# terminusdb-labs/parallel-hnsw

Hardware: AMD Instinct MI355X
Metric: queries/sec at recall@10≥0.95 on 1M×768 f32 (higher is better)
Workload: dtype f32

## Files before the change

### parallel_hnsw_amd/csrc/api.hip

```cpp
#include <hip/hip_runtime.h>

#include <algorithm>
#include <atomic>
#include <cmath>
#include <cstdarg>
#include <cstdio>
#include <cstring>
#include <new>
#include <stdexcept>
#include <vector>

#include "exact_slices.h"
#include "phnsw_internal.h"

static thread_local std::string g_err;

void ph_set_error(const char *fmt, ...) {
  char buf[1024];
  va_list ap;
  va_start(ap, fmt);
  vsnprintf(buf, sizeof(buf), fmt, ap);
  va_end(ap);
  g_err = buf;
}
// ... 674 lines not shown
      int rc = ph_layer_anchor_pos(mix->store, mix->layers[a.n_layers - 1]);
      if (rc) return rc;
      a.probe_pos = mix->layers[a.n_layers - 1].pos;
    }
  }
#endif
#ifdef PH_VISITED_PROBE
  {
    static unsigned long long *vprobe_dev = nullptr;
    if (!vprobe_dev) {
      PH_HIP(hipMalloc(&vprobe_dev, 130 * sizeof(unsigned long long)));
      PH_HIP(hipMemset(vprobe_dev, 0, 130 * sizeof(unsigned long long)));
    } else {
      unsigned long long h[130];
      PH_HIP(hipDeviceSynchronize());
      PH_HIP(hipMemcpy(h, vprobe_dev, sizeof(h), hipMemcpyDeviceToHost));
      for (int k = 0; k < 2; k++) {
        unsigned long long n = 0, sum = 0, run = 0;
        for (int b = 0; b < 64; b++) n += h[64 * k + b], sum += h[64 * k + b] * (64ull * b + 32ull);
        if (!n) continue;
        fprintf(stderr, "[visited probe] %s: %llu walks, mean ~%.0f ids, past the LDS load limit: %.4f; ids < 64*(b+1) for",
                k ? "bottom layer" : "upper gathered layers", n, (double)sum / (double)n, (double)h[128 + k] / (double)n);
        for (int b = 0; b < 64; b++) {
          run += h[64 * k + b];
          if (h[64 * k + b]) fprintf(stderr, " b%d:%.4f", b, (double)run / (double)n);
        }
        fprintf(stderr, "\n");
      }
      PH_HIP(hipMemset(vprobe_dev, 0, 130 * sizeof(unsigned long long)));
    }
    a.vprobe_out = vprobe_dev;
  }
#endif
  return 0;
}

int ph_search_device(const phnsw_index *ix, const PhSearchCall &c) {
  phnsw_index *mix = const_cast<phnsw_index *>(ix);
  const uint64_t nq = c.nq;
  const uint32_t knn_mode = c.knn_mode, out_stride = c.out_stride;
  uint32_t *const out_index = c.out_index;
  const hipStream_t stream = c.stream;
  if (ph_store_converted(ix->store) && (knn_mode || out_index || c.hint || c.out_hit)) {
    return ph_search_only_unsupported(ix->store, knn_mode ? "knn / threshold_nn" : (out_index ? "search_instrumented" : "build search"));
  }
  PhSearchArgs a;
  fill_args(ix, c, a);
  if (ix->dbg_order && ix->dbg_order_n == nq) a.order = ix->dbg_order;
  std::lock_guard<std::mutex> g(mix->ws_mutex);
  if (!mix->totals) {
    PH_HIP(hipMalloc(&mix->totals, 16));
    PH_HIP(hipMemset(mix->totals, 0, 16));
  }
  a.totals = mix->totals;
  PhWorkspace &ws = mix->ws[mix->ws_next & 1];
  mix->ws_last = mix->ws_next & 1;
  mix->ws_next++;
  int rc = ph_workspace_ensure(ix, ws, std::max(a.ef, a.cap_max), c.ovf_cap ? c.ovf_cap : default_ovf_cap(a.ef));
  if (rc) return rc;
  const uint32_t T = (knn_mode || out_index) ? 0u : ph_tiny_layer_count(ix, a.n_layers, a.ef);
  uint32_t first_big = a.n_layers;
  for (uint32_t l = std::max(1u, T); l < a.n_layers; l++)
    if (ph_layer_own_launch(ix->layers[l].n_nodes, ph_row_bytes(ix->store))) {
      first_big = l;
      break;
    }
// ... 337 lines not shown
    return PHNSW_E_INVALID;
  }
  PhFilter f;
  int rc = ph_filter_check(ix, filter_dev, filter_stride_words, 0u, call, &f);
  if (rc) return rc;
  if (!f.words) f.words = ix->default_filter;
  PH_HIP(hipSetDevice(ix->store->device));
  return ph_filter_count(ix, f, nbitmaps, out_count_dev, (hipStream_t)stream);
} catch (...) { return ph_caught(); }

extern "C" int phnsw_debug_last_tiny_table(const phnsw_index *ix, float *out_host, uint64_t cap_floats, uint32_t *npos,
                                           uint32_t *tn, uint32_t *stride, int *g) try {
  if (!ix) return PHNSW_E_INVALID;
  phnsw_index *mix = const_cast<phnsw_index *>(ix);
  std::lock_guard<std::mutex> lock(mix->ws_mutex);
  PhWorkspace &ws = mix->ws[mix->ws_last];
  if (!ws.timed || !ws.d_tiny || !ws.tiny_d) {
    ph_set_error("the last search on this index made no dense table");
    return PHNSW_E_INVALID;
  }
  const uint64_t need = (uint64_t)ws.tiny_last_npos * ws.tiny_last_stride;
  if (npos) *npos = ws.tiny_last_npos;
  if (tn) *tn = ws.tiny_last_tn;
  if (stride) *stride = ws.tiny_last_stride;
  if (g) *g = ws.tiny_table_g;
  if (out_host) {
    if (cap_floats < need) {
      ph_set_error("phnsw_debug_last_tiny_table: %llu floats needed", (unsigned long long)need);
      return PHNSW_E_INVALID;
    }
    PH_HIP(hipSetDevice(ix->store->device));
    PH_HIP(hipEventSynchronize(ws.ev1));
    PH_HIP(hipMemcpy(out_host, ws.tiny_d, need * 4u, hipMemcpyDeviceToHost));
  }
  return 0;
} catch (...) { return ph_caught(); }

extern "C" int phnsw_debug_layer_pos(phnsw_index *ix, uint32_t lft, uint32_t *out_host) try {
  if (lft >= ix->layers.size() || !ix->layers[lft].pos) return PHNSW_E_INVALID;
  PH_HIP(hipMemcpy(out_host, ix->layers[lft].pos, (size_t)ix->layers[lft].n_nodes * 4, hipMemcpyDeviceToHost));
  return 0;
} catch (...) { return ph_caught(); }

extern "C" int phnsw_debug_set_order(phnsw_index *ix, const uint32_t *order_dev, uint64_t n) try {
  ix->dbg_order = order_dev;
  ix->dbg_order_n = n;
  return 0;
} catch (...) { return ph_caught(); }

extern "C" int phnsw_index_counters(const phnsw_index *ix, uint64_t *n_dist, uint64_t *n_hops) try {
  if (!ix) return PHNSW_E_INVALID;
  unsigned long long h[2] = {0, 0};
  if (ix->totals) {
    PH_HIP(hipSetDevice(ix->store->device));
    PH_HIP(hipDeviceSynchronize());
    PH_HIP(hipMemcpy(h, ix->totals, 16, hipMemcpyDeviceToHost));
  }
  if (n_dist) *n_dist = h[0];
  if (n_hops) *n_hops = h[1];
  return 0;
} catch (...) { return ph_caught(); }

extern "C" int phnsw_last_search_kernel_ms(const phnsw_index *ix, float *ms) try {
  if (!ix || !ms) return PHNSW_E_INVALID;
  phnsw_index *mix = const_cast<phnsw_index *>(ix);
  std::lock_guard<std::mutex> g(mix->ws_mutex);
// ... 340 lines not shown
```

### parallel_hnsw_amd/csrc/phnsw_internal.h

```cpp
#pragma once
#include <hip/hip_runtime.h>
#include <stdint.h>
#include <stdlib.h>

#include <mutex>
#include <string>
#include <vector>

#include "../../include/phnsw.h"

#define PH_EMPTY32 0xFFFFFFFFu
#define PH_FMAX 3.4028234663852886e38f
#define PH_MAX_LAYERS 24
#define PH_WAVE 64
#define PH_MAX_DISPATCH 24
#define PH_DENSE_SPLIT_MIN 2048u
#define PH_TINY_MAX_NODES 8192u
#define PH_TINY_LDS_NODES 1024u
#define PH_TINY_MAX_LAYERS 8

void ph_set_error(const char *fmt, ...);
int ph_caught() noexcept;
int ph_hip_fail(hipError_t e, const char *what, const char *file, int line);
#define PH_HIP(x)                                                       \
// ... 59 lines not shown
};

struct phnsw_store {
  int device = 0;
  int kind = PH_ROWS_F32;
  float *rows = nullptr;
  uint8_t *codes = nullptr;
  uint16_t *codes16 = nullptr;
  phnsw_store *centroid_store = nullptr;
  phnsw_index *centroid_index = nullptr;
  phnsw_search_params quantized_search = {0, 0, 0};
  float *codebook = nullptr;
  uint32_t pq_m = 0, pq_ksub = 0, pq_dsub = 0;
  uint32_t pq_table_f16 = 0;
  void *packed = nullptr;
  uint32_t packed_stride = 0;
  float *anchors = nullptr;
  uint32_t *anchor_rank = nullptr;
  uint32_t n_anchors = 0;
  bool owns_rows = true;
  uint64_t n = 0;
  uint32_t dim = 0, ld = 0;
  int metric = 0;
  int refcount = 1;
};

struct PhTinyPrepKey {
  bool valid = false;
  uint64_t nodes_epoch = 0;
  uint32_t T = 0, tn = 0;
  const void *nodes[PH_TINY_MAX_LAYERS] = {}, *nbrs[PH_TINY_MAX_LAYERS] = {}, *vec2node = nullptr;
  uint32_t n[PH_TINY_MAX_LAYERS] = {}, W[PH_TINY_MAX_LAYERS] = {};
  uint64_t links[PH_TINY_MAX_LAYERS] = {};
};
struct PhTinyPackKey {
  bool valid = false;
  uint64_t nodes_epoch = 0;
  const void *vecs = nullptr, *tnodes = nullptr;
  uint32_t ld = 0, tn = 0, nv = 0;
};

struct PhWorkspace {
  uint32_t *visited = nullptr;
  uint64_t visited_words = 0;
  uint2 *ovf = nullptr;
  uint32_t ovf_cap = 0;
  uint32_t n_slots = 0;
  uint32_t *counter = nullptr;
  hipEvent_t ev0 = nullptr, ev1 = nullptr;
  hipEvent_t evc = nullptr;
  bool timed = false;
  void *pq_tables = nullptr;
  size_t pq_tables_bytes = 0;
  uint32_t *okey = nullptr, *okey_sorted = nullptr, *oiota = nullptr, *oorder = nullptr;
  void *sort_tmp = nullptr;
  size_t sort_tmp_bytes = 0;
  uint32_t order_cap = 0;
  float *tiny_d = nullptr;
  size_t tiny_d_bytes = 0;
  uint32_t *tiny_nbr = nullptr;
  size_t tiny_nbr_bytes = 0;
  uint32_t *tiny_member = nullptr;
  size_t tiny_member_bytes = 0;
  float4 *tiny_pq = nullptr, *tiny_pn = nullptr;
  size_t tiny_pq_bytes = 0, tiny_pn_bytes = 0;
  PhTinyPrepKey tiny_prep_key;
  PhTinyPackKey tiny_pack_key;
  int tiny_table_g = 0;
  uint32_t tiny_last_npos = 0, tiny_last_tn = 0, tiny_last_stride = 0;
  uint2 *dense_ovf = nullptr;
  size_t dense_ovf_bytes = 0;
  uint32_t *ovf_s = nullptr;
  size_t ovf_s_cap = 0;
  uint32_t *park_ids = nullptr;
  float *park_d = nullptr;
  size_t park_ids_bytes = 0, park_d_bytes = 0;
  hipEvent_t evd[PH_MAX_DISPATCH + 1] = {};
  unsigned long long *dtotals = nullptr;
  uint32_t n_dispatch = 0;
  uint32_t n_chunks = 0;
  int cus = 0;
  uint32_t d_lo[PH_MAX_DISPATCH] = {}, d_hi[PH_MAX_DISPATCH] = {};
  bool d_tiny = false;
};

struct PhBuildTable {
  float *D = nullptr;
  size_t bytes = 0;
  size_t cap = 0;
  const uint32_t *qnodes = nullptr, *tnodes = nullptr;
  uint32_t qn = 0, tn = 0, T = 0, stride = 0;
  uint32_t lo_alloc = 0, hi_alloc = 0, lo = 0, hi = 0;
  uint64_t epoch = 0;
};
struct PhRowHint {
  const uint32_t *qnodes;
// ... 88 lines not shown
  void *pq_tables;
  uint32_t pq_table_bytes;
  uint32_t layer_lo, layer_hi;
  uint32_t *out_key;
  const uint32_t *key_pos;
  uint32_t dense_only, after_dense;
  const uint32_t *dense_flag;
  uint2 *dense_ovf;
  uint32_t dense_ovf_cap;
#ifdef PH_CELL_PROBE
  const uint32_t *probe_pos;
  unsigned long long *probe_out;
#endif
#ifdef PH_VISITED_PROBE
  unsigned long long *vprobe_out;
#endif
  uint32_t vis_slots, vis_limit, vis_off;
  const uint32_t *order;
  uint32_t seg;
  uint32_t *out_hit;
  uint32_t *out_index;
  uint32_t *ovf_s;
  uint32_t tiny_layers, tiny_n, tiny_stride;
  const float *tiny_d;
  const uint32_t *tiny_nbr;
  const uint32_t *tiny_member;
  uint32_t tiny_rows, tiny_row_first;
  const uint32_t *tiny_row_map;
  uint32_t tiny_off[PH_TINY_MAX_LAYERS];
  const uint32_t *label_of, *label_want;
  uint32_t collect_k, collect_flags;
  uint32_t *collect_ids;
  float *collect_d;
};

uint32_t ph_default_ovf_cap(uint32_t ef);
hipError_t ph_timed_malloc(void **p, size_t bytes);
hipError_t ph_timed_free(void *p);
#ifndef PH_RAW_ALLOC
#define hipMalloc(p, n) ph_timed_malloc((void **)(p), (n))
#define hipFree(p) ph_timed_free((void *)(p))
#endif
static inline long long env_ll(const char *name) {
  const char *e = getenv(name);
  return e ? atoll(e) : 0;
}
static inline uint32_t grid1(uint64_t items) {
  const uint64_t blocks = (items + 255u) / 256u;
  return (uint32_t)(blocks < (1u << 16) ? blocks : (1u << 16));
}
int ph_stream_beside(hipStream_t other, hipStream_t *io);
hipError_t ph_pool_alloc(void **p, size_t bytes);
void ph_pool_free(void *p);
void ph_pool_trim(void);
void ph_layer_free(PhLayerHost &l);
void ph_pending_free(phnsw_index *ix);
void ph_host_stages_free(phnsw_index *ix);
int ph_layer_upload(phnsw_index *ix, const uint32_t *nodes, const uint32_t *neighbors, uint32_t n, uint32_t W,
                    PhLayerHost *out);
struct PhSearchCall {
  const float *queries;
  uint32_t ldq;
  const uint32_t *qids, *exclude;
  uint64_t nq;
  const phnsw_search_params *sp;
  uint32_t upto;
// ... 234 lines not shown
```

### parallel_hnsw_amd/csrc/search_kernels.h

```cpp
#pragma once
#include <hip/hip_runtime.h>

#include <algorithm>
#include <cstdio>
#include <cstdlib>
#include <cstring>

#include "phnsw_internal.h"

#include "phnsw_device.h"

#ifdef PH_HOP_PROFILE
#define PH_TICK(k)                                   \
  {                                                  \
    asm volatile("s_waitcnt vmcnt(0) lgkmcnt(0)");   \
    const uint64_t t_now = wall_clock64();           \
    tprof[k] += t_now - t_last;                      \
    t_last = t_now;                                  \
  }
#else
#define PH_TICK(k)
#endif

template <bool BIG>
// ... 43 lines not shown
  constexpr int CAP = CAPC * 64;
  constexpr int FM = FILT & (PH_FM_BITMAP | PH_FM_LABEL);
  constexpr bool COLLECT = (FILT & PH_FM_COLLECT) != 0;
  constexpr int TAILF = COLLECT ? PH_FM_NONE : FM;
  uint32_t *Cid = smem;
  float *Cd = (float *)(smem + CAP);
  uint32_t *Qid = smem + 2 * CAP;
  float *Qd = (float *)(smem + 3 * CAP);
  if constexpr (BIG) {
    Qid = a.big_q + (uint64_t)blockIdx.x * 2u * a.cap_max;
    Qd = (float *)(Qid + a.cap_max);
  }
  uint32_t *S = smem + 4 * CAP;
  float *dist_lds = (float *)(smem + 5 * CAP + 64);
  if (Dist::GLOBAL_TABLE) dist_lds = (float *)((char *)a.pq_tables + (size_t)blockIdx.x * a.pq_table_bytes);
  const uint32_t T = (a.tiny_layers && a.tiny_member[a.tiny_n] == 0u) ? a.tiny_layers : 0u;
  const bool tiny_lds_row = a.tiny_n <= a.tiny_lds_nodes;
  float *Dl = (float *)(smem + 5 * CAP + 64);
  uint32_t *Vl = smem + 5 * CAP + 64 + (tiny_lds_row ? a.tiny_stride : 0u);
  const uint32_t tiny_words = (a.tiny_n + 31u) / 32u;

  const uint32_t lane = threadIdx.x;
  const uint64_t lt = lanemask_lt(lane);
  constexpr bool DENSE_ONLY = dist_is_none<Dist>::value;
  const bool table_ok = (a.dense_only || a.after_dense) ? a.dense_flag[0] == 0u : true;
  if (DENSE_ONLY && !table_ok) return;
  const uint32_t layer_lo = a.after_dense ? (table_ok ? a.after_dense : 0u) : a.layer_lo;
  uint32_t *vis = a.visited + (uint64_t)blockIdx.x * a.visited_words;
  uint2 *ovf = DENSE_ONLY ? a.dense_ovf + (uint64_t)blockIdx.x * a.dense_ovf_cap : a.ovf + (uint64_t)blockIdx.x * a.ovf_cap;
  const uint32_t ovf_cap = DENSE_ONLY ? a.dense_ovf_cap : a.ovf_cap;
  uint32_t *const Qs = S;
  uint32_t *const ovf_s = INSTR ? a.ovf_s + (uint64_t)blockIdx.x * a.ovf_cap : nullptr;
  uint32_t *const H = smem + a.vis_off;
  const uint32_t hslots = (BIG || INSTR || !vis_lds_policy<CAPC, Dist>::value) ? 0u : a.vis_slots;
  for (uint32_t i = lane; i < hslots; i += 64) H[i] = PH_EMPTY32;

  uint32_t seg_cur = 0, seg_done = 0;
  if (a.order) {
    uint32_t xcc;
    asm volatile("s_getreg_b32 %0, hwreg(HW_REG_XCC_ID)" : "=s"(xcc));
    seg_cur = (xcc & 15u) & 7u;
  }

  for (;;) {
    uint32_t q = 0, qpos = 0;
    if (!a.order) {
      if (lane == 0) q = atomicAdd(a.counter, 1u);
      q = rfl32(q);
      if (q >= a.nq) break;
      qpos = q;
    } else {
      for (;;) {
        uint32_t p = 0;
        if (lane == 0) p = atomicAdd(a.counter + seg_cur * 16u, 1u);
        p = rfl32(p);
        const uint32_t base = seg_cur * a.seg;
        const uint32_t len = base >= a.nq ? 0u : min(a.seg, a.nq - base);
        if (p < len) {
          qpos = base + p;
          q = a.order[qpos];
          break;
        }
        seg_cur = (seg_cur + 1u) & 7u;
        if (++seg_done == 8u) {
          q = PH_EMPTY32;
          break;
        }
      }
// ... 49 lines not shown
      klen = min(kk, klen + (uint32_t)__popcll(em));
      return true;
    };
    uint32_t n_dist = 0, n_hops = 0, err = ST_OK;
    uint32_t index_distance = 0xFFFFFFFFu;
    uint32_t n_tab = 0;
    uint32_t n_dist0 = 0, n_hops0 = 0;
    uint32_t clen = 0;
    uint32_t ef = a.ef;
    bool big_written = false;

    if (layer_lo) {
      clen = a.out_len[q];
#pragma unroll
      for (int c = 0; c < CAPC; c++) {
        uint32_t i = lane + 64u * c;
        if (i < clen) {
          Cid[i] = a.out_ids[(uint64_t)q * a.ef + i];
          Cd[i] = a.out_d[(uint64_t)q * a.ef + i];
        }
      }
      if (a.out_stats) {
        n_dist = a.out_stats[2 * (uint64_t)q];
        n_hops = a.out_stats[2 * (uint64_t)q + 1];
      }
      n_dist0 = n_dist;
      n_hops0 = n_hops;
    } else if (!a.knn_mode) {
      uint32_t entry = a.layers[0].nodes[0];
      float d0;
      if constexpr (DENSE_ONLY) {
        const PhLayerDev TLy = a.layers[a.tiny_layers - 1];
        const uint32_t tid = TLy.vec2node ? TLy.vec2node[entry] : entry;
        d0 = (a.tiny_d + trow * a.tiny_stride)[tid < a.tiny_n ? tid : 0u];
      } else {
        d0 = dist.batch(a.dist, 1ull, entry, lane);
      }
      d0 = __uint_as_float(rl32(__float_as_uint(d0), 0));
      n_dist = 1;
      if (lane == 0) {
        Cid[0] = entry;
        Cd[0] = d0;
      }
      clen = 1;
    }
    const float *Dg = a.tiny_d + trow * a.tiny_stride;
    if (T) {
      if (tiny_lds_row)
        for (uint32_t i = lane; i < a.tiny_n; i += 64) Dl[i] = Dg[i];
      for (uint32_t i = lane; i < tiny_words; i += 64) Vl[i] = 0u;
    }
    queue_sync<BIG>();

    for (uint32_t li = a.knn_mode ? last_layer : layer_lo; li < layer_hi && err == ST_OK; li++) {
      PhLayerDev L = a.layers[li];
      const bool tl = li < T;
      if (tl) {
        const PhLayerDev TLy = a.layers[T - 1];
        L.n_nodes = a.tiny_n;
        L.nodes = TLy.nodes;
        L.vec2node = TLy.vec2node;
        L.neighbors = a.tiny_nbr + a.tiny_off[li];
      }
      const bool identity = L.vec2node == nullptr;
      bool hv = hslots && !tl;
      uint32_t hn = 0;
      auto visit = [&](uint32_t id, bool valid) -> bool {
        if (hv && hn + (uint32_t)__popcll(__ballot(valid)) > a.vis_limit) {
          for (uint32_t i = lane; i < hslots; i += 64) {
            const uint32_t o = H[i];
            if (o != PH_EMPTY32) {
              atomicOr(&vis[o >> 5], 1u << (o & 31));
              H[i] = PH_EMPTY32;
            }
          }
          wait_vm0();
          hv = false;
        }
        if (hv) {
          const bool f = vis_insert(H, hslots, id, valid);
          hn += (uint32_t)__popcll(__ballot(f));
          return f;
        }
        if (!valid) return false;
        const uint32_t bit = 1u << (id & 31);
        return !(atomicOr(&vis[id >> 5], bit) & bit);
      };
      uint32_t qlen;
      if (a.knn_mode) {
        if (lane == 0) {
          Qid[0] = qnode;
          Qd[0] = 0.0f;
        }
        visit(qnode, lane == 0);
        qlen = 1;
// ... 111 lines not shown
            uint32_t id = __hip_atomic_load(&ovf[i].x, __ATOMIC_RELAXED, __HIP_MEMORY_SCOPE_AGENT);
            if (!(id & EXPF)) {
              uint32_t db = __hip_atomic_load(&ovf[i].y, __ATOMIC_RELAXED, __HIP_MEMORY_SCOPE_AGENT);
              uint64_t k = mkkey(__uint_as_float(db), id);
              if (k < best) {
                best = k;
                bi = i;
              }
            }
          }
#pragma unroll
          for (int s = 32; s >= 1; s >>= 1) {
            uint64_t o = ((uint64_t)__shfl_xor((uint32_t)(best >> 32), s) << 32) | __shfl_xor((uint32_t)best, s);
            uint32_t oi = __shfl_xor(bi, s);
            if (o < best) {
              best = o;
              bi = oi;
            }
          }
          if (best == KEY_NONE) break;
          cur = (uint32_t)best & IDM;
          if (lane == 0)
            __hip_atomic_store(&ovf[bi].x, cur | EXPF, __ATOMIC_RELAXED, __HIP_MEMORY_SCOPE_AGENT);
          pop = -1 - (int)bi;
        }
        uint32_t cur_s = 0;
        if constexpr (INSTR) cur_s = pop >= 0 ? Qs[pop] : ovf_s[(uint32_t)(-1 - pop)];
        cur &= IDM;
        n_hops++;
        PH_TICK(0)

        uint32_t nb = PH_EMPTY32;
        if (lane < L.W) nb = L.neighbors[(uint64_t)cur * L.W + lane];
        if constexpr (Dist::EARLY) {
          const bool valid = nb < L.n_nodes;
          uint32_t v = 0;
          if (valid) v = identity ? nb : L.nodes[nb];
          dist.prefetch(a.dist, valid, v, lane);
        }
        PH_TICK(1)
        bool fresh = false;
        if (tl) {
          if (nb < L.n_nodes) {
            uint32_t bit = 1u << (nb & 31);
            fresh = !(atomicOr(&Vl[nb >> 5], bit) & bit);
          }
        } else {
          fresh = visit(nb, nb < L.n_nodes);
        }
        const uint64_t fm = __ballot(fresh);
        const uint32_t m = __popcll(fm);
        n_dist += m;
        if (tl) n_tab += m;
#ifdef PH_CELL_PROBE
        if (probing) {
          uint32_t dd = 0xFFFFFFFFu;
          if (fresh) {
            const int d0 = (int)a.probe_pos[nb] - (int)probe_p0;
            dd = (uint32_t)(d0 < 0 ? -d0 : d0);
          }
#pragma unroll
          for (int k = 0; k < 10; k++) probe_cnt[k] += __popcll(__ballot(fresh && dd <= (k ? (1u << (k - 1)) : 0u)));
          probe_cnt[10] += m;
        }
#endif
        PH_TICK(2)
        uint32_t cvec = 0;
        bool cq = false;
        if constexpr (COLLECT) {
          if (li == last_layer && fresh) {
            cvec = identity ? nb : L.nodes[nb];
            cq = cvec != excl && passes(cvec);
          }
        }

        float myd;
        if (tl) {
          myd = 0.f;
          if (fresh) myd = tiny_lds_row ? Dl[nb] : Dg[nb];
        } else if constexpr (Dist::EARLY) {
          myd = dist.finish(a.dist, fm, lane);
        } else {
          uint32_t vid = 0;
          if (fresh) vid = identity ? nb : L.nodes[nb];
          myd = dist.batch(a.dist, fm, vid, lane);
        }

        PH_TICK(3)
        const uint64_t key = fresh ? mkkey(myd, nb) : KEY_NONE;
        uint32_t my_s = 0;
        if constexpr (INSTR) {
          uint32_t rank_all = 0;
          uint64_t remf = fm;
          while (remf) {
            const int j = __builtin_ctzll(remf);
            remf &= remf - 1;
            rank_all += (rl64(key, j) < key) ? 1u : 0u;
          }
          my_s = cur_s + rank_all + 1u;
        }
        const bool full = qlen == ef;
        const float dtail = full ? Qd[ef - 1] : PH_FMAX;
        const uint64_t tailkey = full ? mkkey(dtail, Qid[ef - 1]) : KEY_NONE;
        const bool ins = fresh && key < tailkey && myd <= PH_FMAX;
        const uint64_t im = __ballot(ins);
        uint32_t pos = 0, pos_min = 0xFFFFFFFFu, newpos = 0xFFFFFFFFu;
        bool did = im != 0;
        if (!im && m >= 2) did = __ballot(fresh && myd == dtail) != 0;
        if (im) {
          uint32_t rank = 0, greater = 0;
          bool first_pass = true;
          const int c_top = (int)((qlen - 1u) >> 6);
// ... 265 lines not shown
      for (int c = 0; c < CAPC; c++) {
        uint32_t j = lane + 64u * c;
        bool has = j < blen;
        bv[c] = has ? Qid[j] : PH_EMPTY32;
        bd[c] = has ? Qd[j] : PH_FMAX;
        bpos[c] = PH_EMPTY32;
        if (has) {
          uint32_t la = lds_lower_bound(Cid, Cd, clen, mkkey(bd[c], bv[c]));
          uint32_t dupb = la < clen ? S[la] : S[CAP];
          if (la == clen) dupb = dups;
          bpos[c] = j + (la - dupb);
        }
      }
      queue_sync<BIG>();
#pragma unroll
      for (int c = 0; c < CAPC; c++) {
        if (cpos[c] < ef) {
          Cid[cpos[c]] = ci[c];
          Cd[cpos[c]] = cd[c];
        }
        if (bpos[c] < ef) {
          Cid[bpos[c]] = bv[c];
          Cd[bpos[c]] = bd[c];
        }
      }
      clen = min(ef, clen - dups + blen);
      queue_sync<BIG>();
    }

    if (err != ST_OK) {
      if (!DENSE_ONLY)
        for (uint64_t w = lane; w < a.visited_words; w += 64) vis[w] = 0u;
      for (uint32_t i = lane; i < hslots; i += 64) H[i] = PH_EMPTY32;
      wait_vm0();
      clen = 0;
      kq = KEY_NONE;
      klen = 0;
    }
    if (TAILF && (a.filter_flags & PHNSW_FILTER_STRICT) && layer_hi == a.n_layers && !big_written) {
      uint32_t sv[CAPC];
      float sd[CAPC];
      uint32_t spos[CAPC];
      uint32_t kept = 0;
#pragma unroll
      for (int c = 0; c < CAPC; c++) {
        const uint32_t i = lane + 64u * c;
        const bool has = i < clen;
        sv[c] = has ? Cid[i] : 0u;
        sd[c] = has ? Cd[i] : PH_FMAX;
        bool keep = false;
        if (has) keep = passes(sv[c]);
        const uint64_t km = __ballot(keep);
        spos[c] = keep ? kept + __popcll(km & lt) : PH_EMPTY32;
        kept += __popcll(km);
      }
      queue_sync<BIG>();
#pragma unroll
      for (int c = 0; c < CAPC; c++) {
        if (spos[c] != PH_EMPTY32) {
          Cid[spos[c]] = sv[c];
          Cd[spos[c]] = sd[c];
        }
      }
      clen = kept;
      queue_sync<BIG>();
    }
    if constexpr (COLLECT) {
      const uint32_t kk = a.collect_k;
      if (lane < kk) {
        a.collect_ids[(uint64_t)q * kk + lane] = lane < klen ? (uint32_t)kq : PH_EMPTY32;
        a.collect_d[(uint64_t)q * kk + lane] = lane < klen ? unfkey((uint32_t)(kq >> 32)) : PH_FMAX;
// ... 188 lines not shown
```

### parallel_hnsw_amd/csrc/tiny.hip

```cpp
#include <hip/hip_runtime.h>

#include <algorithm>
#include <cstdlib>
#include <cstring>

#include "phnsw_device.h"

struct PhTinyPrepArgs {
  PhLayerDev layers[PH_TINY_MAX_LAYERS];
  uint32_t T, tiny_n;
  uint32_t off[PH_TINY_MAX_LAYERS];
  uint32_t *nbr;
  uint32_t *member;
};

__global__ void ph_tiny_prep_kernel(PhTinyPrepArgs p) {
  const uint32_t l = blockIdx.y;
  const PhLayerDev L = p.layers[l], TL = p.layers[p.T - 1];
  for (uint32_t i = blockIdx.x * blockDim.x + threadIdx.x; i < L.n_nodes; i += gridDim.x * blockDim.x) {
    const uint32_t vid = L.nodes[i];
    const uint32_t t = TL.vec2node ? TL.vec2node[vid] : vid;
    if (t >= p.tiny_n) {
      p.member[p.tiny_n] = 1u;
      continue;
    }
    atomicOr(&p.member[t], 1u << l);
    for (uint32_t k = 0; k < L.W; k++) {
      const uint32_t nb = L.neighbors[(uint64_t)i * L.W + k];
      uint32_t tn = PH_EMPTY32;
      if (nb < L.n_nodes) {
        const uint32_t v2 = L.nodes[nb];
        tn = TL.vec2node ? TL.vec2node[v2] : v2;
        if (tn >= p.tiny_n) {
          p.member[p.tiny_n] = 1u;
          tn = PH_EMPTY32;
        }
      }
      p.nbr[p.off[l] + (uint64_t)t * L.W + k] = tn;
    }
  }
}

struct PhTinyTableArgs {
  PhDistArgs dist;
  const float *queries;
  uint32_t ldq;
  const uint32_t *qids;
  const uint32_t *order;
  uint32_t npos;
  const uint32_t *tnodes;
  uint32_t tiny_n, stride;
  float *D;
  uint32_t rows_per_slice;
  uint32_t dbg;
};

template <int M>
__device__ __forceinline__ float fold2(float A, float B, uint32_t lane) {
#ifdef PH_FOLD_GENERIC
  const bool hi = (lane & M) != 0;
  const float own = hi ? B : A, other = hi ? A : B;
  return own + __shfl_xor(other, M);
#else
  if constexpr (M == 32) {
    auto r = __builtin_amdgcn_permlane32_swap(__float_as_uint(A), __float_as_uint(B), false, false);
    return __uint_as_float(r[0]) + __uint_as_float(r[1]);
  } else if constexpr (M == 16) {
    auto r = __builtin_amdgcn_permlane16_swap(__float_as_uint(A), __float_as_uint(B), false, false);
// ... 347 lines not shown
  for (uint32_t s = 0; s < steps; s++) {
    __syncthreads();
    lq[0] = q0;
    lq[32u * ROW16] = q1;
    ln[0] = n0;
    ln[32u * ROW16] = n1;
    __syncthreads();
    if (s + 1u < steps) {
      const uint32_t o = (s + 1u) * KS16;
      q0 = gq[o];
      q1 = gq[half + o];
      n0 = gn[o];
      n1 = gn[half + o];
    }
#pragma unroll
    for (uint32_t j = 0; j < KS16 / 2u; j++) acc = __builtin_amdgcn_mfma_i32_32x32x32_i8(A[2u * j], B[2u * j], acc, 0, 0, 0);
  }
  const uint32_t r = (2u * nt + (w >> 1)) * 32u + (lane & 31u);
  const float sr = a.sn[r];
#pragma unroll
  for (int v = 0; v < 16; v++) {
    const uint32_t p = (2u * qt + (w & 1u)) * 32u + 8u * (v / 4) + 4u * (lane >> 5) + (v & 3);
    if (p < a.npos && r < a.tiny_n) a.D[(uint64_t)p * a.stride + r] = ph_i8q_distance(a.sq[p], sr, acc[v], a.metric);
  }
}


void ph_tiny_free(PhWorkspace &ws) {
  ws.tiny_prep_key = PhTinyPrepKey();
  ws.tiny_pack_key = PhTinyPackKey();
  if (ws.tiny_d) hipFree(ws.tiny_d);
  if (ws.tiny_nbr) hipFree(ws.tiny_nbr);
  if (ws.tiny_member) hipFree(ws.tiny_member);
  if (ws.tiny_pq) hipFree(ws.tiny_pq);
  if (ws.tiny_pn) hipFree(ws.tiny_pn);
  ws.tiny_pq = ws.tiny_pn = nullptr;
  ws.tiny_pq_bytes = ws.tiny_pn_bytes = 0;
  ws.tiny_d = nullptr;
  ws.tiny_nbr = ws.tiny_member = nullptr;
  ws.tiny_d_bytes = ws.tiny_nbr_bytes = ws.tiny_member_bytes = 0;
}

static bool tiny_mfma_shape(int metric, uint32_t ld) {
  return metric != PHNSW_METRIC_L2 && (ld == 256u || ld == 768u || ld == 1536u) && !getenv("PHNSW_TINY_VALU");
}

static int table_beside_mode() {
  const char *e = getenv("PHNSW_TABLE_BESIDE");
  if (!e || !strcmp(e, "auto")) return 2;
  return atoi(e) > 0 ? 1 : 0;
}
static bool tiny_keep_off() { return getenv("PHNSW_NO_TINY_KEEP") != nullptr; }
static size_t tiny_mfma_lds(int nv, int g) { return (size_t)2 * 4 * g * nv * 64 * sizeof(float4); }

bool ph_tiny_matrix_cores(const phnsw_index *ix) {
  return ix->store->kind == PH_ROWS_I8Q || tiny_mfma_shape(ix->store->metric, ix->store->ld);
}

uint32_t ph_tiny_layer_count(const phnsw_index *ix, uint32_t n_layers, uint32_t ef) {
  const bool off = getenv("PHNSW_NO_TINY") != nullptr;
  if (off || (!ph_store_f32(ix->store) && !ph_store_converted(ix->store)) || !ph_chunk_count(ix->store->ld / 4)) return 0;
  const uint64_t per_ef = ph_tiny_matrix_cores(ix) ? 80ull : 48ull;
  uint64_t cap = std::min<uint64_t>(PH_TINY_MAX_NODES, per_ef * ef);
  if (const char *e = getenv("PHNSW_TINY_MAX"))
    if (atoi(e) > 0) cap = std::min<uint64_t>(PH_TINY_MAX_NODES, (uint64_t)atoi(e));
  uint32_t T = 0;
  while (T < n_layers && T < PH_TINY_MAX_LAYERS && ix->layers[T].n_nodes <= cap) T++;
  return T;
}

static uint32_t tiny_stride_of(uint32_t n) { return (n + 63u) / 64u * 64u; }

uint64_t ph_tiny_max_positions(const phnsw_index *ix, uint32_t n_layers, uint32_t ef) {
  uint32_t T = ph_tiny_layer_count(ix, n_layers, ef);
  if (!T) return 0;
  uint64_t budget = 4ull << 30;
  if (const char *e = getenv("PHNSW_TINY_TABLE_BYTES"))
    if (atoll(e) > 0) budget = (uint64_t)atoll(e);
  return std::max<uint64_t>(64, budget / ((uint64_t)tiny_stride_of(ix->layers[T - 1].n_nodes) * 4u));
}

size_t ph_tiny_beside_lds(const phnsw_index *ix, const PhSearchArgs &a) {
  if (!a.tiny_layers || a.tiny_rows || !table_beside_mode()) return 0;
  if (ix->store->kind == PH_ROWS_I8Q) return PH_I8T_LDS;
  const uint32_t nv4 = a.dist.nv4;
  if (!tiny_mfma_shape(ix->store->metric, nv4 * 4u)) return 0;
  return tiny_mfma_lds((int)(nv4 / 64u), 1);
}

size_t ph_tiny_lds_bytes(const PhSearchArgs &a) {
  if (!a.tiny_layers) return 0;
  return (a.tiny_n <= a.tiny_lds_nodes ? (size_t)a.tiny_stride * 4u : 0u) + (size_t)((a.tiny_n + 31u) / 32u + 1u) * 4u;
}

template <class T>
static hipError_t grow(T **p, size_t *have, size_t need) {
  if (*have >= need) return hipSuccess;
  if (*p) ph_timed_free(*p);
  *p = nullptr;
  *have = 0;
  hipError_t e = ph_timed_malloc((void **)p, need);
  if (e == hipSuccess) *have = need;
  return e;
}

static bool same_key(const PhTinyPrepKey &a, const PhTinyPrepKey &b) {
  if (!a.valid || !b.valid || a.nodes_epoch != b.nodes_epoch || a.T != b.T || a.tn != b.tn || a.vec2node != b.vec2node) return false;
  for (uint32_t l = 0; l < a.T; l++)
    if (a.nodes[l] != b.nodes[l] || a.nbrs[l] != b.nbrs[l] || a.n[l] != b.n[l] || a.W[l] != b.W[l] || a.links[l] != b.links[l])
      return false;
  return true;
}

static int tiny_prep_graph(const phnsw_index *ix, PhWorkspace &ws, PhSearchArgs &a, uint32_t T, uint32_t tn, hipStream_t stream,
                           bool *kept = nullptr) {
  if (kept) *kept = false;
  PhTinyPrepArgs p;
  memset(&p, 0, sizeof(p));
  p.T = T;
  p.tiny_n = tn;
  PhTinyPrepKey key;
  key.valid = !tiny_keep_off();
  key.nodes_epoch = ix->nodes_epoch;
  key.T = T;
  key.tn = tn;
  key.vec2node = a.layers[T - 1].vec2node;
  size_t nbr_words = 0;
  for (uint32_t l = 0; l < T; l++) {
    p.layers[l] = a.layers[l];
    p.off[l] = (uint32_t)nbr_words;
    a.tiny_off[l] = (uint32_t)nbr_words;
    nbr_words += (size_t)tn * a.layers[l].W;
    key.nodes[l] = a.layers[l].nodes;
    key.nbrs[l] = a.layers[l].neighbors;
    key.n[l] = a.layers[l].n_nodes;
    key.W[l] = a.layers[l].W;
    key.links[l] = ix->layers[l].links_epoch;
  }
  const uint32_t *nbr_was = ws.tiny_nbr, *member_was = ws.tiny_member;
  if (grow(&ws.tiny_nbr, &ws.tiny_nbr_bytes, nbr_words * 4u) != hipSuccess ||
      grow(&ws.tiny_member, &ws.tiny_member_bytes, (size_t)(PH_TINY_MAX_NODES + 1u) * 4u) != hipSuccess) {
    (void)hipGetLastError();
    ws.tiny_prep_key.valid = false;
    return 1;
  }
  if (ws.tiny_nbr == nbr_was && ws.tiny_member == member_was && same_key(key, ws.tiny_prep_key)) {
    if (kept) *kept = true;
    return 0;
  }
  ws.tiny_prep_key = key;
  p.nbr = ws.tiny_nbr;
  p.member = ws.tiny_member;
  PH_HIP(hipMemsetAsync(ws.tiny_nbr, 0xFF, nbr_words * 4u, stream));
  PH_HIP(hipMemsetAsync(ws.tiny_member, 0, (size_t)(tn + 1u) * 4u, stream));
  hipLaunchKernelGGL(ph_tiny_prep_kernel, dim3((tn + 255u) / 256u, T), dim3(256), 0, stream, p);
  PH_HIP(hipGetLastError());
  return 0;
}

template <class R>
static void tiny_table_valu(int nv, dim3 grid, hipStream_t stream, const PhTinyTableArgs &t) {
  switch (nv) {
    case 1: hipLaunchKernelGGL((ph_tiny_table_kernel<1, 8, R>), grid, dim3(256), 0, stream, t); break;
    case 3: hipLaunchKernelGGL((ph_tiny_table_kernel<3, 8, R>), grid, dim3(256), 0, stream, t); break;
    default: hipLaunchKernelGGL((ph_tiny_table_kernel<6, 4, R>), grid, dim3(256), 0, stream, t); break;
  }
}

static int tiny_table_i8q(const phnsw_index *ix, PhWorkspace &ws, const PhDistArgs &dist, const float *queries, uint32_t ldq,
                          const uint32_t *qids, const uint32_t *order, uint32_t npos, const uint32_t *tnodes, uint32_t tn,
                          uint32_t stride, float *D, hipStream_t stream, bool *kept) {
  const uint32_t qtiles = (npos + 63u) / 64u, ntiles = (tn + 63u) / 64u;
  const uint32_t kpad = (dist.ld + PH_I8T_KS - 1u) / PH_I8T_KS * PH_I8T_KS;
  const size_t row_bytes = (size_t)kpad + 4u;
  const float4 *pn_was = ws.tiny_pn;
  if (grow(&ws.tiny_pq, &ws.tiny_pq_bytes, (size_t)qtiles * 64u * row_bytes) != hipSuccess ||
      grow(&ws.tiny_pn, &ws.tiny_pn_bytes, (size_t)ntiles * 64u * row_bytes) != hipSuccess) {
    (void)hipGetLastError();
    ws.tiny_pack_key.valid = false;
    return 1;
  }
  PhTinyPackKey key;
  key.valid = !tiny_keep_off();
  key.nodes_epoch = ix->nodes_epoch;
  key.vecs = dist.rows.base;
  key.tnodes = tnodes;
  key.ld = dist.ld;
  key.tn = tn;
// ... 166 lines not shown
  return tiny_table(ix, ws, ph_dist_args(ix->store), queries, ldq, qids, nullptr, npos, tnodes, tn, tiny_stride_of(tn), D, stream,
                    2, kept);
}

int ph_tiny_table_chunk_ordered(const phnsw_index *ix, PhWorkspace &ws, const float *queries, uint32_t ldq,
                                const uint32_t *qids, const uint32_t *order, uint32_t npos, const uint32_t *tnodes,
                                uint32_t tn, float *D, hipStream_t stream, bool *kept) {
  return tiny_table(ix, ws, ph_dist_args(ix->store), queries, ldq, qids, order, npos, tnodes, tn, tiny_stride_of(tn), D, stream,
                    2, kept);
}

int ph_tiny_prepare(const phnsw_index *ix, PhWorkspace &ws, PhSearchArgs &a, uint32_t max_layers, hipStream_t stream) {
  a.tiny_layers = 0;
  a.tiny_rows = 0;
  if (a.knn_mode || a.layer_lo) return 0;
  uint32_t T = std::min(ph_tiny_layer_count(ix, a.n_layers, a.ef), max_layers);
  if (!T) return 0;
  const uint32_t tn = ix->layers[T - 1].n_nodes, stride = tiny_stride_of(tn), npos = a.nq;
  if ((uint64_t)npos > ph_tiny_max_positions(ix, a.n_layers, a.ef)) return 0;
  if (grow(&ws.tiny_d, &ws.tiny_d_bytes, std::max<size_t>((size_t)npos * stride * 4u, 1u << 20)) != hipSuccess) {
    (void)hipGetLastError();
    return 0;
  }
  const int mode = table_beside_mode();
  bool beside = mode == 1;
  if (mode == 2) {
    const PhWorkspace &other = &ws == &ix->ws[0] ? ix->ws[1] : ix->ws[0];
    if ((&ws == &ix->ws[0] || &ws == &ix->ws[1]) && other.timed && other.ev1) {
      beside = hipEventQuery(other.ev1) == hipErrorNotReady;
      (void)hipGetLastError();
    }
  }
  bool prep_kept = false, pack_kept = false;
  int rc = tiny_prep_graph(ix, ws, a, T, tn, stream, &prep_kept);
  if (rc) return rc < 0 ? rc : 0;
  rc = tiny_table(ix, ws, a.dist, a.queries, a.ldq, a.qids, a.order, npos, a.layers[T - 1].nodes, tn, stride, ws.tiny_d, stream,
                  beside ? 1 : 2, &pack_kept);
  if (rc) return rc < 0 ? rc : 0;
  if (getenv("PHNSW_VERBOSE")) {
    if (ws.tiny_table_g)
      fprintf(stderr, "[phnsw] dense table: %u positions x %u nodes on the matrix cores, G = %d (%s), graph %s, node operand %s\n",
              npos, tn, ws.tiny_table_g, beside ? "beside the other workspace's launch" : "alone",
              prep_kept ? "kept" : "prepared", pack_kept ? "kept" : "packed");
    else
      fprintf(stderr, "[phnsw] dense table: %u positions x %u nodes on the vector units, graph %s\n", npos, tn,
              prep_kept ? "kept" : "prepared");
  }
  ws.tiny_last_npos = npos;
  ws.tiny_last_tn = tn;
  ws.tiny_last_stride = stride;
  a.tiny_layers = T;
  a.tiny_n = tn;
  a.tiny_lds_nodes = PH_TINY_LDS_NODES;
  a.tiny_stride = stride;
  a.tiny_d = ws.tiny_d;
  a.tiny_nbr = ws.tiny_nbr;
  a.tiny_member = ws.tiny_member;
  return 0;
}


void ph_build_table_free(phnsw_index *ix) {
  for (PhBuildTable &b : ix->bt)
    if (b.D) ph_timed_free(b.D);
  ix->bt.clear();
  for (auto &sp : ix->bt_spare) ph_timed_free(sp.first);
  ix->bt_spare.clear();
}
static void build_table_drop(phnsw_index *ix, PhBuildTable &b) {
  if (b.D) ix->bt_spare.emplace_back(b.D, b.cap);
  b.D = nullptr;
  b.bytes = b.cap = 0;
  b.lo = b.hi = b.lo_alloc = b.hi_alloc = 0;
}
static void build_table_recycle(phnsw_index *ix) {
  for (PhBuildTable &b : ix->bt) build_table_drop(ix, b);
  ix->bt.clear();
}
static float *build_table_buffer(phnsw_index *ix, size_t bytes, size_t *cap) {
  int best = -1;
  for (size_t i = 0; i < ix->bt_spare.size(); i++)
    if (ix->bt_spare[i].second >= bytes && ix->bt_spare[i].second <= 2 * bytes &&
        (best < 0 || ix->bt_spare[i].second < ix->bt_spare[(size_t)best].second))
      best = (int)i;
  if (best >= 0) {
    float *p = ix->bt_spare[(size_t)best].first;
    *cap = ix->bt_spare[(size_t)best].second;
    ix->bt_spare.erase(ix->bt_spare.begin() + best);
    return p;
  }
// ... 40 lines not shown
    found = &ix->bt.back();
    found->epoch = ix->nodes_epoch;
    found->qnodes = h.qnodes;
    found->qn = h.qn;
  }
  PhBuildTable &B = *found;
  const uint32_t need_lo = h.contiguous ? h.first : 0u, need_hi = h.contiguous ? h.first + h.count : h.qn;
  if (need_hi > h.qn || need_lo >= need_hi) return 0;
  const bool same = B.D && B.tnodes == tnodes && B.tn == tn && B.T == T;
  if (B.D && !same) build_table_drop(ix, B);
  if (!h.contiguous && !(B.D && B.lo <= need_lo && B.hi >= need_hi)) return 0;
  if (!B.D || need_lo < B.lo_alloc || need_hi > B.hi_alloc) {
    if (B.D && (need_lo > B.lo_alloc || need_hi < B.hi_alloc)) return 0;
    build_table_drop(ix, B);
    const size_t bytes = (size_t)(need_hi - need_lo) * stride * 4u;
    B.D = build_table_buffer(ix, bytes, &B.cap);
    if (!B.D) return 0;
    B.bytes = bytes;
    B.qnodes = h.qnodes;
    B.qn = h.qn;
    B.tnodes = tnodes;
    B.tn = tn;
    B.T = T;
    B.stride = stride;
    B.lo_alloc = need_lo;
    B.hi_alloc = need_hi;
    B.lo = B.hi = need_lo;
    B.epoch = ix->nodes_epoch;
  }
  auto fill = [&](uint32_t lo, uint32_t hi) -> int {
    const uint32_t PIECE = 131072u;
    for (uint32_t at = lo; at < hi; at += PIECE) {
      const uint32_t cnt = std::min(PIECE, hi - at);
      int rc = tiny_table(ix, ws, a.dist, nullptr, 0, h.qnodes + at, nullptr, cnt, tnodes, tn, stride,
                          B.D + (size_t)(at - B.lo_alloc) * stride, stream);
      if (rc) return rc;
    }
    return 0;
  };
  int rc = 0;
  if (B.lo == B.hi) {
    rc = fill(need_lo, need_hi);
    if (!rc) B.lo = need_lo, B.hi = need_hi;
  } else {
    if (need_lo < B.lo) {
      rc = fill(need_lo, B.lo);
      if (!rc) B.lo = need_lo;
    }
    if (!rc && need_hi > B.hi) {
      rc = fill(B.hi, need_hi);
      if (!rc) B.hi = need_hi;
    }
  }
  if (rc) return rc < 0 ? rc : 0;
  rc = tiny_prep_graph(ix, ws, a, T, tn, stream);
  if (rc) return rc < 0 ? rc : 0;
  a.tiny_layers = T;
  a.tiny_n = tn;
  a.tiny_lds_nodes = PH_TINY_LDS_NODES;
  a.tiny_stride = stride;
  a.tiny_d = B.D;
  a.tiny_rows = 1;
  a.tiny_row_first = B.lo_alloc;
  a.tiny_row_map = h.vec2node;
  a.tiny_nbr = ws.tiny_nbr;
  a.tiny_member = ws.tiny_member;
  *used = true;
  return 0;
}
```

Before: 1.053 million.

## Reorder dense-table columns by in-degree and stage hot columns in LDS hash space

Ranks the small upper-layer nodes by upper-layer membership and in-degree, then permutes the dense distance table's columns into that order. Neighbor words are packed with the column index in their high bits. During search, the hottest prefix of each query's table row is copied into the otherwise idle visited-hash LDS region, so most table lookups hit LDS instead of global memory. This adds an order kernel and a word-rewrite kernel to graph prep, plus extra hash clears. It also assumes node ids and column ranks fit in 16 bits.

```diff
diff --git a/parallel_hnsw_amd/csrc/api.hip b/parallel_hnsw_amd/csrc/api.hip
--- a/parallel_hnsw_amd/csrc/api.hip
+++ b/parallel_hnsw_amd/csrc/api.hip
@@ -730,6 +730,26 @@
     a.vprobe_out = vprobe_dev;
   }
 #endif
+#ifdef PH_TABLE_HOT_PROBE
+  {
+    static unsigned long long *hprobe_dev = nullptr;
+    if (!hprobe_dev) {
+      PH_HIP(hipMalloc(&hprobe_dev, 4 * sizeof(unsigned long long)));
+      PH_HIP(hipMemset(hprobe_dev, 0, 4 * sizeof(unsigned long long)));
+    } else {
+      unsigned long long h[4];
+      PH_HIP(hipDeviceSynchronize());
+      PH_HIP(hipMemcpy(h, hprobe_dev, sizeof(h), hipMemcpyDeviceToHost));
+      if (h[0] + h[1] + h[2] + h[3])
+        fprintf(stderr, "[table hot probe] lookups above the table layer: %llu LDS, %llu global; in the table layer: %llu LDS, %llu global; "
+                        "LDS share %.4f / %.4f / all %.4f\n",
+                h[0], h[1], h[2], h[3], (double)h[0] / (double)std::max(1ull, h[0] + h[1]),
+                (double)h[2] / (double)std::max(1ull, h[2] + h[3]), (double)(h[0] + h[2]) / (double)(h[0] + h[1] + h[2] + h[3]));
+      PH_HIP(hipMemset(hprobe_dev, 0, 4 * sizeof(unsigned long long)));
+    }
+    a.hprobe_out = hprobe_dev;
+  }
+#endif
   return 0;
 }
 
@@ -1133,6 +1153,36 @@
     PH_HIP(hipSetDevice(ix->store->device));
     PH_HIP(hipEventSynchronize(ws.ev1));
     PH_HIP(hipMemcpy(out_host, ws.tiny_d, need * 4u, hipMemcpyDeviceToHost));
+    std::vector<uint32_t> col(ws.tiny_last_tn);
+    std::vector<float> row(ws.tiny_last_tn);
+    PH_HIP(hipMemcpy(col.data(), ws.tiny_col, col.size() * 4u, hipMemcpyDeviceToHost));
+    for (uint32_t p = 0; p < ws.tiny_last_npos; p++) {
+      float *r = out_host + (uint64_t)p * ws.tiny_last_stride;
+      for (uint32_t t = 0; t < ws.tiny_last_tn; t++) row[t] = r[col[t] < ws.tiny_last_tn ? col[t] : t];
+      std::copy(row.begin(), row.end(), r);
+    }
+  }
+  return 0;
+} catch (...) { return ph_caught(); }
+
+extern "C" int phnsw_debug_last_tiny_columns(const phnsw_index *ix, uint32_t *out_host, uint32_t cap, uint32_t *tn) try {
+  if (!ix) return PHNSW_E_INVALID;
+  phnsw_index *mix = const_cast<phnsw_index *>(ix);
+  std::lock_guard<std::mutex> lock(mix->ws_mutex);
+  PhWorkspace &ws = mix->ws[mix->ws_last];
+  if (!ws.timed || !ws.d_tiny || !ws.tiny_col) {
+    ph_set_error("the last search on this index made no dense table");
+    return PHNSW_E_INVALID;
+  }
+  if (tn) *tn = ws.tiny_last_tn;
+  if (out_host) {
+    if (cap < ws.tiny_last_tn) {
+      ph_set_error("phnsw_debug_last_tiny_columns: %u entries needed", ws.tiny_last_tn);
+      return PHNSW_E_INVALID;
+    }
+    PH_HIP(hipSetDevice(ix->store->device));
+    PH_HIP(hipEventSynchronize(ws.ev1));
+    PH_HIP(hipMemcpy(out_host, ws.tiny_col, (size_t)ws.tiny_last_tn * 4u, hipMemcpyDeviceToHost));
   }
   return 0;
 } catch (...) { return ph_caught(); }
diff --git a/parallel_hnsw_amd/csrc/phnsw_internal.h b/parallel_hnsw_amd/csrc/phnsw_internal.h
--- a/parallel_hnsw_amd/csrc/phnsw_internal.h
+++ b/parallel_hnsw_amd/csrc/phnsw_internal.h
@@ -115,6 +115,7 @@
   const void *nodes[PH_TINY_MAX_LAYERS] = {}, *nbrs[PH_TINY_MAX_LAYERS] = {}, *vec2node = nullptr;
   uint32_t n[PH_TINY_MAX_LAYERS] = {}, W[PH_TINY_MAX_LAYERS] = {};
   uint64_t links[PH_TINY_MAX_LAYERS] = {};
+  bool by_degree = true;
 };
 struct PhTinyPackKey {
   bool valid = false;
@@ -145,6 +146,7 @@
   size_t tiny_nbr_bytes = 0;
   uint32_t *tiny_member = nullptr;
   size_t tiny_member_bytes = 0;
+  uint32_t *tiny_col = nullptr;
   float4 *tiny_pq = nullptr, *tiny_pn = nullptr;
   size_t tiny_pq_bytes = 0, tiny_pn_bytes = 0;
   PhTinyPrepKey tiny_prep_key;
@@ -299,6 +301,11 @@
   uint32_t collect_k, collect_flags;
   uint32_t *collect_ids;
   float *collect_d;
+  const uint32_t *tiny_col;
+  uint32_t tiny_hot_cols;
+#ifdef PH_TABLE_HOT_PROBE
+  unsigned long long *hprobe_out;
+#endif
 };
 
 uint32_t ph_default_ovf_cap(uint32_t ef);
diff --git a/parallel_hnsw_amd/csrc/search_kernels.h b/parallel_hnsw_amd/csrc/search_kernels.h
--- a/parallel_hnsw_amd/csrc/search_kernels.h
+++ b/parallel_hnsw_amd/csrc/search_kernels.h
@@ -99,8 +99,11 @@
   uint32_t *const Qs = S;
   uint32_t *const ovf_s = INSTR ? a.ovf_s + (uint64_t)blockIdx.x * a.ovf_cap : nullptr;
   uint32_t *const H = smem + a.vis_off;
-  const uint32_t hslots = (BIG || INSTR || !vis_lds_policy<CAPC, Dist>::value) ? 0u : a.vis_slots;
+  constexpr bool HASH = !BIG && !INSTR && vis_lds_policy<CAPC, Dist>::value;
+  const uint32_t hslots = HASH ? a.vis_slots : 0u;
   for (uint32_t i = lane; i < hslots; i += 64) H[i] = PH_EMPTY32;
+  float *const Hf = (HASH && !tiny_lds_row) ? (float *)H : Dl;
+  const uint32_t hot = T ? min(min(tiny_lds_row ? a.tiny_n : hslots, a.tiny_n), a.tiny_hot_cols) : 0u;
 
   uint32_t seg_cur = 0, seg_done = 0;
   if (a.order) {
@@ -216,7 +219,7 @@
       if constexpr (DENSE_ONLY) {
         const PhLayerDev TLy = a.layers[a.tiny_layers - 1];
         const uint32_t tid = TLy.vec2node ? TLy.vec2node[entry] : entry;
-        d0 = (a.tiny_d + trow * a.tiny_stride)[tid < a.tiny_n ? tid : 0u];
+        d0 = (a.tiny_d + trow * a.tiny_stride)[tid < a.tiny_n ? a.tiny_col[tid] : 0u];
       } else {
         d0 = dist.batch(a.dist, 1ull, entry, lane);
       }
@@ -229,9 +232,12 @@
       clen = 1;
     }
     const float *Dg = a.tiny_d + trow * a.tiny_stride;
+    bool h_holds_row = false;
     if (T) {
-      if (tiny_lds_row)
-        for (uint32_t i = lane; i < a.tiny_n; i += 64) Dl[i] = Dg[i];
+      if (layer_lo < T) {
+        for (uint32_t i = lane; i < hot; i += 64) Hf[i] = Dg[i];
+        if constexpr (HASH) h_holds_row = hot && !tiny_lds_row;
+      }
       for (uint32_t i = lane; i < tiny_words; i += 64) Vl[i] = 0u;
     }
     queue_sync<BIG>();
@@ -245,6 +251,10 @@
         L.nodes = TLy.nodes;
         L.vec2node = TLy.vec2node;
         L.neighbors = a.tiny_nbr + a.tiny_off[li];
+      }
+      if (HASH && h_holds_row && !tl) {
+        for (uint32_t i = lane; i < hot; i += 64) H[i] = PH_EMPTY32;
+        h_holds_row = false;
       }
       const bool identity = L.vec2node == nullptr;
       bool hv = hslots && !tl;
@@ -422,6 +432,11 @@
 
         uint32_t nb = PH_EMPTY32;
         if (lane < L.W) nb = L.neighbors[(uint64_t)cur * L.W + lane];
+        uint32_t col = 0;
+        if (tl) {
+          col = nb >> 16;
+          nb &= 0xFFFFu;
+        }
         if constexpr (Dist::EARLY) {
           const bool valid = nb < L.n_nodes;
           uint32_t v = 0;
@@ -467,7 +482,17 @@
         float myd;
         if (tl) {
           myd = 0.f;
-          if (fresh) myd = tiny_lds_row ? Dl[nb] : Dg[nb];
+          if (fresh) myd = col < hot ? Hf[col] : Dg[col];
+#ifdef PH_TABLE_HOT_PROBE
+          {
+            const uint32_t in_lds = (uint32_t)__popcll(__ballot(fresh && col < hot));
+            if (lane == 0 && m) {
+              const uint32_t k = li + 1u == T ? 2u : 0u;
+              atomicAdd(&a.hprobe_out[k], (unsigned long long)in_lds);
+              atomicAdd(&a.hprobe_out[k + 1u], (unsigned long long)(m - in_lds));
+            }
+          }
+#endif
         } else if constexpr (Dist::EARLY) {
           myd = dist.finish(a.dist, fm, lane);
         } else {
@@ -799,11 +824,14 @@
       if (!DENSE_ONLY)
         for (uint64_t w = lane; w < a.visited_words; w += 64) vis[w] = 0u;
       for (uint32_t i = lane; i < hslots; i += 64) H[i] = PH_EMPTY32;
+      h_holds_row = false;
       wait_vm0();
       clen = 0;
       kq = KEY_NONE;
       klen = 0;
     }
+    if (HASH && h_holds_row)
+      for (uint32_t i = lane; i < hot; i += 64) H[i] = PH_EMPTY32;
     if (TAILF && (a.filter_flags & PHNSW_FILTER_STRICT) && layer_hi == a.n_layers && !big_written) {
       uint32_t sv[CAPC];
       float sd[CAPC];
diff --git a/parallel_hnsw_amd/csrc/tiny.hip b/parallel_hnsw_amd/csrc/tiny.hip
--- a/parallel_hnsw_amd/csrc/tiny.hip
+++ b/parallel_hnsw_amd/csrc/tiny.hip
@@ -12,7 +12,35 @@
   uint32_t off[PH_TINY_MAX_LAYERS];
   uint32_t *nbr;
   uint32_t *member;
+  uint32_t *indeg;
+  uint32_t *col;
+  uint32_t *cnodes;
+  uint32_t nbr_words;
 };
+
+__device__ __forceinline__ uint32_t tiny_col_key(const PhTinyPrepArgs &p, uint32_t t) {
+  const uint32_t upper = p.T >= 2u ? (p.member[t] >> (p.T - 2u)) & 1u : 1u;
+  const uint32_t deg = p.indeg ? min(p.indeg[t], 0x3FFFu) : 0u;
+  return ((upper ^ 1u) << 27) | ((0x3FFFu - deg) << 13) | t;
+}
+__global__ __launch_bounds__(256) void ph_tiny_order_kernel(PhTinyPrepArgs p) {
+  __shared__ uint32_t keys[PH_TINY_MAX_NODES];
+  for (uint32_t i = threadIdx.x; i < p.tiny_n; i += 256u) keys[i] = tiny_col_key(p, i);
+  __syncthreads();
+  const uint32_t t = blockIdx.x * 256u + threadIdx.x;
+  if (t >= p.tiny_n) return;
+  const uint32_t mine = keys[t];
+  uint32_t rank = 0;
+  for (uint32_t i = 0; i < p.tiny_n; i++) rank += keys[i] < mine ? 1u : 0u;
+  p.col[t] = rank;
+  p.cnodes[rank] = p.layers[p.T - 1].nodes[t];
+}
+__global__ void ph_tiny_word_kernel(PhTinyPrepArgs p) {
+  for (uint32_t i = blockIdx.x * blockDim.x + threadIdx.x; i < p.nbr_words; i += gridDim.x * blockDim.x) {
+    const uint32_t t = p.nbr[i];
+    if (t != PH_EMPTY32) p.nbr[i] = (p.col[t] << 16) | t;
+  }
+}
 
 __global__ void ph_tiny_prep_kernel(PhTinyPrepArgs p) {
   const uint32_t l = blockIdx.y;
@@ -34,6 +62,8 @@
         if (tn >= p.tiny_n) {
           p.member[p.tiny_n] = 1u;
           tn = PH_EMPTY32;
+        } else if (p.indeg && l == p.T - 1u) {
+          atomicAdd(&p.indeg[tn], 1u);
         }
       }
       p.nbr[p.off[l] + (uint64_t)t * L.W + k] = tn;
@@ -447,6 +477,8 @@
   if (ws.tiny_d) hipFree(ws.tiny_d);
   if (ws.tiny_nbr) hipFree(ws.tiny_nbr);
   if (ws.tiny_member) hipFree(ws.tiny_member);
+  if (ws.tiny_col) hipFree(ws.tiny_col);
+  ws.tiny_col = nullptr;
   if (ws.tiny_pq) hipFree(ws.tiny_pq);
   if (ws.tiny_pn) hipFree(ws.tiny_pn);
   ws.tiny_pq = ws.tiny_pn = nullptr;
@@ -464,6 +496,10 @@
   const char *e = getenv("PHNSW_TABLE_BESIDE");
   if (!e || !strcmp(e, "auto")) return 2;
   return atoi(e) > 0 ? 1 : 0;
+}
+static uint32_t tiny_hot_cols() {
+  const char *e = getenv("PHNSW_TINY_HOT_COLS");
+  return e && atoll(e) >= 0 ? (uint32_t)std::min<long long>(atoll(e), PH_TINY_MAX_NODES) : PH_TINY_MAX_NODES;
 }
 static bool tiny_keep_off() { return getenv("PHNSW_NO_TINY_KEEP") != nullptr; }
 static size_t tiny_mfma_lds(int nv, int g) { return (size_t)2 * 4 * g * nv * 64 * sizeof(float4); }
@@ -520,7 +556,9 @@
 }
 
 static bool same_key(const PhTinyPrepKey &a, const PhTinyPrepKey &b) {
-  if (!a.valid || !b.valid || a.nodes_epoch != b.nodes_epoch || a.T != b.T || a.tn != b.tn || a.vec2node != b.vec2node) return false;
+  if (!a.valid || !b.valid || a.nodes_epoch != b.nodes_epoch || a.T != b.T || a.tn != b.tn || a.vec2node != b.vec2node ||
+      a.by_degree != b.by_degree)
+    return false;
   for (uint32_t l = 0; l < a.T; l++)
     if (a.nodes[l] != b.nodes[l] || a.nbrs[l] != b.nbrs[l] || a.n[l] != b.n[l] || a.W[l] != b.W[l] || a.links[l] != b.links[l])
       return false;
@@ -528,7 +566,7 @@
 }
 
 static int tiny_prep_graph(const phnsw_index *ix, PhWorkspace &ws, PhSearchArgs &a, uint32_t T, uint32_t tn, hipStream_t stream,
-                           bool *kept = nullptr) {
+                           bool by_degree, bool *kept = nullptr) {
   if (kept) *kept = false;
   PhTinyPrepArgs p;
   memset(&p, 0, sizeof(p));
@@ -540,6 +578,7 @@
   key.T = T;
   key.tn = tn;
   key.vec2node = a.layers[T - 1].vec2node;
+  key.by_degree = by_degree;
   size_t nbr_words = 0;
   for (uint32_t l = 0; l < T; l++) {
     p.layers[l] = a.layers[l];
@@ -553,10 +592,13 @@
     key.links[l] = ix->layers[l].links_epoch;
   }
   const uint32_t *nbr_was = ws.tiny_nbr, *member_was = ws.tiny_member;
+  size_t col_bytes = ws.tiny_col ? (size_t)3u * PH_TINY_MAX_NODES * 4u : 0u;
   if (grow(&ws.tiny_nbr, &ws.tiny_nbr_bytes, nbr_words * 4u) != hipSuccess ||
-      grow(&ws.tiny_member, &ws.tiny_member_bytes, (size_t)(PH_TINY_MAX_NODES + 1u) * 4u) != hipSuccess) {
+      grow(&ws.tiny_member, &ws.tiny_member_bytes, (size_t)(PH_TINY_MAX_NODES + 1u) * 4u) != hipSuccess ||
+      grow(&ws.tiny_col, &col_bytes, (size_t)3u * PH_TINY_MAX_NODES * 4u) != hipSuccess) {
     (void)hipGetLastError();
     ws.tiny_prep_key.valid = false;
+    ws.tiny_pack_key.valid = false;
     return 1;
   }
   if (ws.tiny_nbr == nbr_was && ws.tiny_member == member_was && same_key(key, ws.tiny_prep_key)) {
@@ -564,11 +606,19 @@
     return 0;
   }
   ws.tiny_prep_key = key;
+  ws.tiny_pack_key.valid = false;
   p.nbr = ws.tiny_nbr;
   p.member = ws.tiny_member;
+  p.col = ws.tiny_col;
+  p.cnodes = ws.tiny_col + PH_TINY_MAX_NODES;
+  p.indeg = by_degree ? ws.tiny_col + 2u * PH_TINY_MAX_NODES : nullptr;
+  p.nbr_words = (uint32_t)nbr_words;
   PH_HIP(hipMemsetAsync(ws.tiny_nbr, 0xFF, nbr_words * 4u, stream));
   PH_HIP(hipMemsetAsync(ws.tiny_member, 0, (size_t)(tn + 1u) * 4u, stream));
+  if (by_degree) PH_HIP(hipMemsetAsync(p.indeg, 0, (size_t)tn * 4u, stream));
   hipLaunchKernelGGL(ph_tiny_prep_kernel, dim3((tn + 255u) / 256u, T), dim3(256), 0, stream, p);
+  hipLaunchKernelGGL(ph_tiny_order_kernel, dim3((tn + 255u) / 256u), dim3(256), 0, stream, p);
+  hipLaunchKernelGGL(ph_tiny_word_kernel, dim3(grid1(nbr_words)), dim3(256), 0, stream, p);
   PH_HIP(hipGetLastError());
   return 0;
 }
@@ -801,10 +851,10 @@
     }
   }
   bool prep_kept = false, pack_kept = false;
-  int rc = tiny_prep_graph(ix, ws, a, T, tn, stream, &prep_kept);
+  int rc = tiny_prep_graph(ix, ws, a, T, tn, stream, true, &prep_kept);
   if (rc) return rc < 0 ? rc : 0;
-  rc = tiny_table(ix, ws, a.dist, a.queries, a.ldq, a.qids, a.order, npos, a.layers[T - 1].nodes, tn, stride, ws.tiny_d, stream,
-                  beside ? 1 : 2, &pack_kept);
+  rc = tiny_table(ix, ws, a.dist, a.queries, a.ldq, a.qids, a.order, npos, ws.tiny_col + PH_TINY_MAX_NODES, tn, stride, ws.tiny_d,
+                  stream, beside ? 1 : 2, &pack_kept);
   if (rc) return rc < 0 ? rc : 0;
   if (getenv("PHNSW_VERBOSE")) {
     if (ws.tiny_table_g)
@@ -825,6 +875,8 @@
   a.tiny_d = ws.tiny_d;
   a.tiny_nbr = ws.tiny_nbr;
   a.tiny_member = ws.tiny_member;
+  a.tiny_col = ws.tiny_col;
+  a.tiny_hot_cols = tiny_hot_cols();
   return 0;
 }
 
@@ -931,13 +983,14 @@
     const uint32_t PIECE = 131072u;
     for (uint32_t at = lo; at < hi; at += PIECE) {
       const uint32_t cnt = std::min(PIECE, hi - at);
-      int rc = tiny_table(ix, ws, a.dist, nullptr, 0, h.qnodes + at, nullptr, cnt, tnodes, tn, stride,
+      int rc = tiny_table(ix, ws, a.dist, nullptr, 0, h.qnodes + at, nullptr, cnt, ws.tiny_col + PH_TINY_MAX_NODES, tn, stride,
                           B.D + (size_t)(at - B.lo_alloc) * stride, stream);
       if (rc) return rc;
     }
     return 0;
   };
-  int rc = 0;
+  int rc = tiny_prep_graph(ix, ws, a, T, tn, stream, false);
+  if (rc) return rc < 0 ? rc : 0;
   if (B.lo == B.hi) {
     rc = fill(need_lo, need_hi);
     if (!rc) B.lo = need_lo, B.hi = need_hi;
@@ -951,8 +1004,6 @@
       if (!rc) B.hi = need_hi;
     }
   }
-  if (rc) return rc < 0 ? rc : 0;
-  rc = tiny_prep_graph(ix, ws, a, T, tn, stream);
   if (rc) return rc < 0 ? rc : 0;
   a.tiny_layers = T;
   a.tiny_n = tn;
@@ -964,6 +1015,8 @@
   a.tiny_row_map = h.vec2node;
   a.tiny_nbr = ws.tiny_nbr;
   a.tiny_member = ws.tiny_member;
+  a.tiny_col = ws.tiny_col;
+  a.tiny_hot_cols = tiny_hot_cols();
   *used = true;
   return 0;
 }
```

Measured after the change: 1.063 million (median of 6 runs). About the same (+1.0%).
